# rongzhao-zhang/EfficientQ

Hardware: AMD Instinct MI355X
Metric: ptq_calibration_throughput (higher is better)
Workload: dtype i8xi8->i32 (exact) for the Gram systems and per-iteration loss convs of the layers with quantised input, f32/f64 elsewhere

## Files before the change

### efficientq_amd/_lib.py

```python
from __future__ import annotations

import ctypes as C
import os

import torch

_HERE = os.path.dirname(os.path.abspath(__file__))
LIB_PATH = os.path.join(_HERE, "libeffq_hip.so")

EFFQ_OK = 0
_ERR_NAMES = {1: "EFFQ_ERR_ARG", 2: "EFFQ_ERR_HIP", 3: "EFFQ_ERR_WORKSPACE", 4: "EFFQ_ERR_NO_DEVICE",
              5: "EFFQ_ERR_NOT_CONVERGED"}


class EffqError(RuntimeError):
    pass


class Geom(C.Structure):
    _fields_ = [(n, C.c_int32) for n in
                ("N", "C1", "C2", "D", "H", "W", "KD", "KH", "KW", "SD", "SH", "SW", "PD", "PH", "PW")]

    def out_dims(self):
        return ((self.D + 2 * self.PD - self.KD) // self.SD + 1,
# ... 79 lines not shown
    "effq_fixed_point_coop_rec": (_I, [_P, _P, _P, _SZ, _I, _D, _D, _D, _I, _P, _P, _P, _P]),
    "effq_fp_check": (_I, [_P, _P, _P]),
    "effq_fp_channels_max_row": (_I, []),
    "effq_fixed_point_channels": (_I, [_P, _P, _P, _I, _I, _I, _D, _I, _P, _P, _P, _P]),
    "effq_fixed_point_channels_proj": (_I, [_P, _P, _P, _I, _I, _I, _D, _I, _P, _P, _P, _P, _F, _P, _P, _P, _I, _I, _D,
                                            _D, _P]),
    "effq_gram_packed_elems": (_SZ, [_I, _I]),
    "effq_gram_pack": (_I, [_P, _P, _I, _I, _P, _P]),
    "effq_gram_unpack": (_I, [_P, _I, _I, _P, _P, _P]),
    "effq_act_quant_backward": (_I, [_P, _P, _I, _P, _P, _P, _SZ, _P, _P]),
    "effq_att_classes_ws_bytes": (_SZ, []),
    "effq_att_classes": (_I, [_P, _LL, _P, _P, _P, C.POINTER(C.c_int32), _P, _P]),
    "effq_prof_enable": (_I, [_I]),
    "effq_prof_count": (_I, []),
    "effq_prof_read": (_I, [_I, C.POINTER(ProfRecord)]),
    "effq_admm_num_inverses": (_I, [_D, _D, _I, _I]),
    "effq_admm_run": (_I, [C.POINTER(AdmmRunArgs)]),
    "effq_admm_select_best": (_I, [_P, _I, _P, _P, _SZ, _SZ, _P, _P, _P, _P]),
    "effq_gram_ws_bytes": (_SZ, [_GP, _I]),
    "effq_gram_accum": (_I, [_P, _P, _P, _GP, _I, _P, _P, _I, _P, _SZ, _P]),
    "effq_gram_plan_query": (_I, [_GP, _I, _IP, _IP, _IP, _IP, _LLP, _IP, _IP]),
    "effq_gram_i8_supported": (_I, [_GP, _I]),
    "effq_gram_i8_ws_bytes": (_SZ, [_GP, _I]),
    "effq_gram_accum_i8": (_I, [_P, _P, _GP, _I, _P, _I, _P, _P, _P, _I, _LL, _P, _P, _I, _P, _SZ, _P]),
    "effq_gram_accum_i8_unw": (_I, [_P, _P, _GP, _I, _P, _I, _P, _P, _P, _I, _LL, _P, _P, _I, _P, _P, _P, _SZ, _P]),
    "effq_gram_i8_plan_query": (_I, [_GP, _I, _LL, _IP, _IP, _IP, _IP, _IP, _IP]),
    "effq_upsample_trilinear": (_I, [_P, _I, _I, _I, _I, _I, _I, _I, _I, _P, _P]),
    "effq_gram_f64_supported": (_I, [_GP, _I]),
    "effq_gram_f64_ws_bytes": (_SZ, [_GP, _I]),
    "effq_gram_f64": (_I, [_P, _P, _GP, _I, _P, _P, _P, _SZ, _P]),
    "effq_gram_f64_plan_query": (_I, [_GP, _I, _IP, _IP, _IP, _IP]),
    "effq_gram_loss_ws_bytes": (_SZ, [_I]),
    "effq_gram_loss": (_I, [_P, _P, _P, _P, _P, _I, _I, _I, _P, _P, _SZ, _P]),
    "effq_packed_bytes": (_SZ, [_SZ, _I]),
    "effq_pack_levels": (_I, [_P, _SZ, _I, _P, _P]),
    "effq_unpack_levels": (_I, [_P, _SZ, _I, _P, _P]),
    "effq_ainv_ld": (_I, [_I]),
    "effq_fp_bracket_export_words": (_SZ, []),
    "effq_fp_bracket_export": (_I, [_P, _SZ, _P, _P, _SZ, _P]),
    "effq_fp_bracket_rebase": (_I, [_P, _P, _SZ, _P]),
    "effq_fp_bracket_import": (_I, [_P, _SZ, _P, _I, _SZ, _P, _P, _SZ, _P]),
    "effq_admm_uses_traj": (_I, [_SZ, _I]),
    "effq_gram_loss_i8_supported": (_I, [_I, _I, _I, _I]),
    "effq_gram_loss_i8_num_planes": (_I, [C.c_longlong]),
    "effq_gram_loss_i8_planes_bytes": (_SZ, [_I, _I, _I]),
    "effq_gram_loss_i8_prepare": (_I, [_P, _I, _I, _P, _I, _I, _P, _P, _P]),
    "effq_gram_loss_i8_ws_bytes": (_SZ, []),
    "effq_gram_loss_i8": (_I, [_P, _I, _P, _P, _P, _P, _P, _P, _P, _I, _I, _I, _I, _I, _I, _P, _P, _SZ, _P]),
    "effq_spd_inverse_ws_bytes": (_SZ, [_I]),
    "effq_spd_inverse": (_I, [_P, _I, _I, _D, _D, _P, _P, _SZ, _P]),
    "effq_spd_inverse_plan": (_I, [_I, _IP, _IP, _IP]),
    "effq_prox_plan_query": (_I, [_I, _I, _IP, _IP, _IP, _IP]),
    "effq_prox_ws_bytes": (_SZ, [_I, _I]),
    "effq_prox_solve": (_I, [_P, _P, _P, _P, _P, _P, _I, _I, _I, _D, _D, _P, _P, _P, _SZ, _P]),
    "effq_prox_solve_shifted": (_I, [_P, _P, _P, _P, _P, _P, _I, _I, _I, _D, _D, _D, _I, _P, _P, _P, _SZ, _P]),
    "effq_admm_presum": (_I, [_P, _P, _P, _SZ, _P]),
    "effq_admm_project_dual": (_I, [_P, _P, _P, _I, _P, _P, _F, _P, _SZ, _P]),
    "effq_conv_i8_supported": (_I, [_GP, _I, _I]),
    "effq_conv_i8s_supported": (_I, [_GP, _I, _I]),
    "effq_conv_i8s_ws_bytes": (_SZ, [_GP, _I, _I]),
    "conv3d_calib_step_i8s": (_I, [_P, _P, _P, _P, _GP, _P, _I, _P, _I, _I, _P, _P, _SZ, _P]),
    "effq_conv_i8_ws_bytes": (_SZ, [_GP]),
    "conv3d_calib_step_i8": (_I, [_P, _P, _P, _P, _GP, _P, _I, _P, _I, _P, _P, _SZ, _P]),
    "effq_conv_i8_out_supported": (_I, [_GP, _I, _I]),
    "conv3d_quant_forward_i8": (_I, [_P, _P, _P, _P, _P, _GP, _P, _I, _P, _I, _P, _P, _P, _SZ, _P]),
    "effq_conv_ws_bytes": (_SZ, [_GP]),
# ... 56 lines not shown
```

### efficientq_amd/csrc/admm_run.hip

```cpp
#include <stdlib.h>
#include <algorithm>
#include <vector>
#include "common.h"
#include "internal.h"
#include "project_dual.h"

namespace effq {

struct ProfRec {
  int kind, iter, loss_kind, c2, n;
  effq_geom geom;
  hipEvent_t e0, e1;
};
static thread_local std::vector<ProfRec> g_prof;
static thread_local int g_prof_every = 0;
enum { PROF_PROX = 1, PROF_FIXED_POINT = 2, PROF_PROJECT = 3, PROF_LOSS = 4, PROF_INVERSE = 5, PROF_WAIT = 6 };

struct ProfScope {
  bool on;
  hipStream_t stream;
  ProfRec rec;
  ProfScope(bool enabled, int kind, int iter, const effq_admm_run_args* a, hipStream_t st) : on(enabled), stream(st) {
    if (!on) return;
    rec.kind = kind;
    rec.iter = iter;
    rec.loss_kind = a->loss_kind;
    rec.c2 = a->c2;
    rec.n = a->n;
    rec.geom = a->geom;
    if (hipEventCreate(&rec.e0) != hipSuccess || hipEventCreate(&rec.e1) != hipSuccess) {
      on = false;
      return;
    }
    (void)hipEventRecord(rec.e0, stream);
  }
  void close() {
    if (!on) return;
    (void)hipEventRecord(rec.e1, stream);
    g_prof.push_back(rec);
    on = false;
  }
};

constexpr int ADMM_MAX_RHOS = 16;

struct RhoPlan {
  int count;
  double rho[ADMM_MAX_RHOS];
  int first_iter[ADMM_MAX_RHOS];
  bool shifted_first;
  bool overflow;
};

static RhoPlan plan_rhos(double rho, double rho_max, int iters, int period) {
  RhoPlan p;
  p.count = 0;
  p.overflow = false;
  double r = rho;
// ... 293 lines not shown
                                        a->alpha_ring + (size_t)it.i * p.c2,
                                        a->w_iters_ring ? a->w_iters_ring + (size_t)it.i * p.c2 : nullptr, a->err_flag,
                                        it.G, it.dual_div, it.next_rhs ? p.bm : nullptr, a->B0, a->W0, p.n, p.bm_ld,
                                        it.rho_next, a->eta, p.s_main);
  else if (kind == FpKind::traj && it.parts != nullptr)
    rc = effq_fixed_point_traj_parts(it.parts, it.parts_n, it.parts_ld, p.c2, nwrow, p.has_b, a->dual, a->wstar, it.bstar,
                                     a->v, a->w_levels, -1.0, 1.0, a->tol, maxit, it.st, a->fp_pred, a->fp_traj_ws,
                                     a->fp_traj_ws_bytes, p.s_main);
  else if (kind == FpKind::traj)
    rc = effq_fixed_point_traj(a->wstar, a->dual, a->v, p.nw, a->w_levels, -1.0, 1.0, a->tol, maxit, it.st, a->fp_pred,
                               a->fp_traj_ws, a->fp_traj_ws_bytes, p.s_main);
  else if (kind == FpKind::bucket)
    rc = effq_fixed_point_bucket_rec(a->wstar, a->dual, a->v, p.nw, a->w_levels, -1.0, 1.0, a->tol, maxit, it.st, a->fp_ws,
                                     a->fp_ws_bytes, rec, p.s_main);
  else if (kind == FpKind::small)
    rc = effq_fixed_point_small_fused(a->wstar, a->dual, a->v, p.nw, a->w_levels, -1.0, 1.0, a->tol, maxit, it.st,
                                      fuse_proj ? &pf : nullptr, p.s_main);
  else
    rc = effq_fixed_point_coop_rec(a->wstar, a->dual, a->v, p.nw, a->w_levels, -1.0, 1.0, a->tol, maxit, it.st, a->red_ws,
                                   rec, p.s_main);
  if (rc != EFFQ_OK) return rc;
  p_fp.close();
  *bm_ready = it.next_rhs;
  if (fuse_proj) return EFFQ_OK;
  ProfScope p_pr(it.prof, PROF_PROJECT, it.i, a, p.s_main);
  rc = effq_project_dual_impl(a->v, a->wstar, it.st, a->w_levels, it.G, a->dual, it.dual_div, it.Gq, p.nw, a->err_flag,
                              nxp, p.s_main);
  if (rc != EFFQ_OK) return rc;
  p_pr.close();
  return EFFQ_OK;
}

static int enqueue_losses(const effq_admm_run_args* a, const AdmmPlan& p, int j0, int i) {
  const int step = a->loss_kind == 5 ? 16 : 1;
  for (int j = j0; j <= i; j += step) {
    const int cnt = (i - j + 1 < step) ? (i - j + 1) : step;
    const float* Gj = a->G_ring + (size_t)j * p.nw;
    const int8_t* Gqj = a->Gq_ring ? a->Gq_ring + (size_t)j * p.nw : nullptr;
    const float* bj = p.has_b ? a->b_ring + (size_t)j * p.c2 : nullptr;
    const effq_fp_state* stj = a->state_ring + j;
    double* sq = a->hist + 2 * (size_t)j;
    const bool prof = g_prof_every > 0 && (a->loss_kind == 5 ? (j / p.loss_group) % 2 == 1 :
                      !(p.rhos.shifted_first && j == 0) && (j % g_prof_every) == g_prof_every / 2);
    ProfScope p_loss(prof, PROF_LOSS, j, a, p.s_loss);
    int rc;
    if (a->loss_kind == 5)
      rc = effq_gram_loss_i8(a->loss_planes, a->loss_nplanes, a->loss_Au, a->loss_Bu, a->loss_syy, Gqj, bj, stj,
                             a->act_alpha_dev, a->act_levels, a->w_levels, p.c2, p.n, p.has_b, cnt, sq, a->conv_ws,
                             a->conv_ws_bytes, p.s_loss);
    else if (a->loss_kind == 1)
      rc = conv3d_calib_step_i8(a->xidx, Gqj, bj, a->y_fp, &a->geom, a->act_alpha_dev, a->act_levels, stj, a->w_levels,
                                sq, a->conv_ws, a->conv_ws_bytes, p.s_loss);
    else if (a->loss_kind == 2)
      rc = conv3d_calib_step_i8s(a->xidx, Gqj, bj, a->y_fp, &a->geom, a->act_alpha_dev, a->act_levels, stj, a->w_levels,
                                 j == 0 ? 1 : 0, sq, a->conv_ws, a->conv_ws_bytes, p.s_loss);
    else if (a->loss_kind == 4)
      rc = effq_gram_loss(a->loss_Au, a->loss_Bu, a->loss_syy, Gj, bj, p.c2, p.n, p.has_b, sq, a->conv_ws,
                          a->conv_ws_bytes, p.s_loss);
    else
      rc = conv3d_quant_calib_step(a->xq, Gj, bj, a->y_fp, nullptr, &a->geom, nullptr, 0, sq, nullptr, a->conv_ws,
                                   a->conv_ws_bytes, p.s_loss);
    if (rc != EFFQ_OK) return rc;
    p_loss.close();
  }
  return EFFQ_OK;
}

}
using namespace effq;

extern "C" {

int effq_admm_uses_traj(size_t nw, int w_levels) {
  constexpr int traj_levels = 4;
  constexpr size_t traj_min = 65536;
  return (w_levels <= traj_levels && nw >= traj_min && nw <= effq_fp_traj_max()) ? 1 : 0;
}

int effq_admm_num_inverses(double rho, double rho_max, int iters, int period) {
  if (!(rho > 0.0) || iters <= 0 || period <= 0) return -1;
  const RhoPlan p = plan_rhos(rho, rho_max, iters, period);
  if (p.overflow) return -1;
  return p.count - (p.shifted_first ? 1 : 0);
}

int effq_admm_run(const effq_admm_run_args* a) {
  AdmmPlan p;
  if (const int rc = admm_plan(a, &p); rc != EFFQ_OK) return rc;
  constexpr int LOSS_EVENTS = 4;
  EventPool events;
  EFFQ_HIP(events.open());
// ... 74 lines not shown

int effq_gram_unpack(const float* buf, int n, int c2, float* A0, float* B0, void* stream) {
  EFFQ_CHECK_ARG(A0 && B0 && buf && n > 0 && c2 > 0);
  size_t blocks = ((size_t)n * n + (size_t)c2 * n + 255) / 256;
  if (blocks > 8192) blocks = 8192;
  hipLaunchKernelGGL(k_gram_unpack, dim3((unsigned)blocks), dim3(256), 0, as_stream(stream), buf, n, c2, A0, B0);
  EFFQ_LAUNCH_CHECK();
  return EFFQ_OK;
}

int effq_prof_enable(int every) {
  for (ProfRec& r : g_prof) {
    (void)hipEventDestroy(r.e0);
    (void)hipEventDestroy(r.e1);
  }
  g_prof.clear();
  g_prof_every = every > 0 ? every : 0;
  return EFFQ_OK;
}

int effq_prof_count(void) { return (int)g_prof.size(); }

int effq_prof_read(int i, effq_prof_record* out) {
  EFFQ_CHECK_ARG(out != nullptr && i >= 0 && i < (int)g_prof.size());
  const ProfRec& r = g_prof[(size_t)i];
  float ms = 0.0f;
  EFFQ_HIP(hipEventElapsedTime(&ms, r.e0, r.e1));
  out->kind = r.kind;
  out->iter = r.iter;
  out->loss_kind = r.loss_kind;
  out->c2 = r.c2;
  out->n = r.n;
  out->geom = r.geom;
  out->ms = ms;
  return EFFQ_OK;
}

int effq_admm_select_best(const double* hist, int iters, const float* G_ring, const float* b_ring, size_t nw, size_t nb,
                          float* best_G, float* best_b, double* best_out, void* stream) {
  EFFQ_CHECK_ARG(hist && G_ring && best_G && best_out && iters > 0 && nw > 0);
  EFFQ_CHECK_ARG((b_ring == nullptr) == (best_b == nullptr));
  size_t blocks = (nw + 255) / 256;
  if (blocks > 1024) blocks = 1024;
  hipLaunchKernelGGL(k_select_best, dim3((unsigned)blocks), dim3(256), 0, as_stream(stream), hist, iters, G_ring, b_ring,
                     nw, nb, best_G, best_b, best_out);
  EFFQ_LAUNCH_CHECK();
  return EFFQ_OK;
}

}
```

### efficientq_amd/csrc/gram_loss.hip

```cpp
#include "common.h"

namespace effq {

constexpr int GL_TB = 64;
constexpr int GL_T = 256;
constexpr int GL_CC = 32;

struct GramLossParams {
  const double* Au;
  const double* Bu;
  const double* syy;
  const float* G;
  const float* b;
  int c2, n, has_bias, nt;
  int ntile, ncross;
  double* partials;
  unsigned int* ticket;
  double* out;
};

__device__ __forceinline__ float gl_g(const GramLossParams& p, int c, int k) {
  const int nw = p.n - p.has_bias;
  if (k < nw) return p.G[(size_t)c * nw + k];
  return (k < p.n && p.b != nullptr) ? p.b[c] : 0.0f;
}

__global__ __launch_bounds__(GL_T) void k_gram_loss(GramLossParams p) {
  __shared__ float gk[GL_CC][GL_TB + 4], gj[GL_CC][GL_TB + 4];
  __shared__ double red_smem[16];
  __shared__ int s_last;
  const int tid = threadIdx.x;
  double part = 0.0;
  if ((int)blockIdx.x < p.ntile) {
    int K = 0, rem = (int)blockIdx.x;
    while (rem >= p.nt - K) {
      rem -= p.nt - K;
      ++K;
    }
    const int J = K + rem;
    const int k0 = K * GL_TB, j0 = J * GL_TB;
    const int tk = (tid >> 4) * 4, tj = (tid & 15) * 4;
    double m[4][4];
#pragma unroll
    for (int a = 0; a < 4; ++a)
#pragma unroll
      for (int b = 0; b < 4; ++b) m[a][b] = 0.0;
    for (int c0 = 0; c0 < p.c2; c0 += GL_CC) {
      __syncthreads();
      for (int e = tid; e < GL_CC * GL_TB; e += GL_T) {
        const int c = e / GL_TB, q = e % GL_TB;
        const bool cok = c0 + c < p.c2;
        gk[c][q] = cok ? gl_g(p, c0 + c, k0 + q) : 0.0f;
        gj[c][q] = cok ? gl_g(p, c0 + c, j0 + q) : 0.0f;
      }
      __syncthreads();
#pragma unroll 4
      for (int c = 0; c < GL_CC; ++c) {
        double a4[4], b4[4];
#pragma unroll
        for (int a = 0; a < 4; ++a) {
          a4[a] = (double)gk[c][tk + a];
          b4[a] = (double)gj[c][tj + a];
        }
#pragma unroll
        for (int a = 0; a < 4; ++a)
#pragma unroll
          for (int b = 0; b < 4; ++b) m[a][b] = __builtin_fma(a4[a], b4[b], m[a][b]);
      }
    }
    double acc = 0.0;
#pragma unroll
    for (int a = 0; a < 4; ++a) {
      const int k = k0 + tk + a;
#pragma unroll
      for (int b = 0; b < 4; ++b) {
        const int j = j0 + tj + b;
        if (k < p.n && j < p.n) acc = __builtin_fma(p.Au[(size_t)k * p.n + j], m[a][b], acc);
      }
    }
    part = (J > K) ? 2.0 * acc : acc;
  } else {
    const int w = (int)blockIdx.x - p.ntile;
    const size_t tot = (size_t)p.c2 * p.n;
    double acc = 0.0;
    for (size_t e = (size_t)w * GL_T + tid; e < tot; e += (size_t)p.ncross * GL_T) {
      const int c = (int)(e / p.n), k = (int)(e % p.n);
      acc = __builtin_fma((double)gl_g(p, c, k), p.Bu[e], acc);
    }
    part = -2.0 * acc;
  }
  double v[1] = {part};
  grid_sum_finish<1>(v, p.partials, p.ticket, p.out, red_smem, &s_last);
  if (s_last && tid == 0) {
    const double loss = p.out[0] + *p.syy;
    p.out[0] = loss;
    p.out[1] = loss;
  }
}

}
using namespace effq;

extern "C" {

size_t effq_gram_loss_ws_bytes(int n) {
  if (n <= 0) return 0;
  const size_t nt = ((size_t)n + GL_TB - 1) / GL_TB;
  return 256 + (nt * (nt + 1) / 2 + 64) * sizeof(double) + 256;
}

int effq_gram_loss(const double* Au, const double* Bu, const double* syy_dev, const float* G, const float* b, int c2, int n,
                   int has_bias, double* sqerr_out, void* ws, size_t ws_bytes, void* stream) {
  EFFQ_CHECK_ARG(Au && Bu && syy_dev && G && sqerr_out && ws && c2 > 0 && n > 0);
  EFFQ_CHECK_ARG(!has_bias || b != nullptr);
  if (ws_bytes < effq_gram_loss_ws_bytes(n)) {
    set_error("gram_loss: workspace %zu < required %zu", ws_bytes, effq_gram_loss_ws_bytes(n));
    return EFFQ_ERR_WORKSPACE;
  }
  GramLossParams p;
  p.Au = Au; p.Bu = Bu; p.syy = syy_dev; p.G = G; p.b = has_bias ? b : nullptr;
  p.c2 = c2; p.n = n; p.has_bias = has_bias ? 1 : 0;
  p.nt = (n + GL_TB - 1) / GL_TB;
  p.ntile = p.nt * (p.nt + 1) / 2;
  size_t nc = ((size_t)c2 * n + (size_t)GL_T * 8 - 1) / ((size_t)GL_T * 8);
  if (nc < 1) nc = 1;
  if (nc > 64) nc = 64;
  p.ncross = (int)nc;
  EFFQ_CHECK_ARG(p.ntile + p.ncross <= RED_MAX_BLOCKS * 16);
  char* base = reinterpret_cast<char*>(ws);
  p.ticket = reinterpret_cast<unsigned int*>(base);
  p.partials = reinterpret_cast<double*>(base + 256);
  p.out = sqerr_out;
  hipLaunchKernelGGL(k_gram_loss, dim3((unsigned)(p.ntile + p.ncross)), dim3(GL_T), 0, as_stream(stream), p);
  EFFQ_LAUNCH_CHECK();
  return EFFQ_OK;
}

}
```

### efficientq_amd/hip_ops.py

```python
from __future__ import annotations

import ctypes as C
import math
from typing import Optional, Tuple

import torch

from . import _lib
from ._lib import Geom, check

ADMM_TOL = 1e-5
FP_BRACKET_MIN = 1 << 18
DP_GATHER_AFTER = 4
DP_GATHER_MAX_BYTES = 128 << 20


def _ptr(t: Optional[torch.Tensor]):
    return None if t is None else C.c_void_p(t.data_ptr())


def to_ndhwc(x: torch.Tensor) -> torch.Tensor:
    return x.permute(0, 2, 3, 4, 1).contiguous()


# ... 423 lines not shown
        return bool(self.lib.effq_gram_f64_supported(C.byref(geom), int(has_bias)))

    def gram_f64(self, x_ndhwc: torch.Tensor, y_ndhwc: torch.Tensor, geom: Geom, has_bias: bool):
        x, y = self._f32(x_ndhwc), self._f32(y_ndhwc)
        _check_shapes(geom, x, y=y)
        n = geom.C1 * geom.KD * geom.KH * geom.KW + int(has_bias)
        Au = torch.empty(n, n, dtype=torch.float64, device=self.device)
        Bu = torch.empty(geom.C2, n, dtype=torch.float64, device=self.device)
        ws = self._workspace("gram_f64", self.lib.effq_gram_f64_ws_bytes(C.byref(geom), int(has_bias)))
        check(self.lib.effq_gram_f64(_ptr(x), _ptr(y), C.byref(geom), int(has_bias), _ptr(Au), _ptr(Bu), _ptr(ws),
                                     ws.numel(), self.stream), "effq_gram_f64")
        return Au, Bu

    def upsample_trilinear(self, x_ndhwc: torch.Tensor, scale) -> torch.Tensor:
        x = self._f32(x_ndhwc)
        N, D, H, W, Cc = (int(i) for i in x.shape)
        sd, sh, sw = (int(i) for i in scale)
        out = torch.empty(N, D * sd, H * sh, W * sw, Cc, dtype=torch.float32, device=self.device)
        check(self.lib.effq_upsample_trilinear(_ptr(x), N, D, H, W, Cc, sd, sh, sw, _ptr(out), self.stream),
              "effq_upsample_trilinear")
        return out

    def gram_loss(self, Au: torch.Tensor, Bu: torch.Tensor, syy: torch.Tensor, G: torch.Tensor, b, sqerr=None):
        c2, n = (int(i) for i in Bu.shape)
        has_b = b is not None
        if (Au.dtype != torch.float64 or Bu.dtype != torch.float64 or syy.dtype != torch.float64 or
                tuple(Au.shape) != (n, n) or G.numel() != c2 * (n - int(has_b))):
            raise _lib.EffqError("gram_loss: operand shapes / dtypes do not match")
        if sqerr is None:
            sqerr = torch.zeros(2, dtype=torch.float64, device=self.device)
        ws = self._workspace("gram_loss", self.lib.effq_gram_loss_ws_bytes(n))
        check(self.lib.effq_gram_loss(_ptr(Au), _ptr(Bu), _ptr(syy), _ptr(self._f32(G)), _ptr(b), c2, n, int(has_b),
                                      _ptr(sqerr), _ptr(ws), ws.numel(), self.stream), "effq_gram_loss")
        return sqerr

    def gram_loss_i8_supported(self, c2: int, n: int, has_b: bool, w_levels: int) -> bool:
        return bool(self.lib.effq_gram_loss_i8_supported(int(c2), int(n), int(has_b), int(w_levels)))

    def gram_loss_i8_planes(self, Au: torch.Tensor, has_b: bool, act_alpha: torch.Tensor, act_levels: int, voxels: int):
        n = int(Au.shape[0])
        P = self.lib.effq_gram_loss_i8_num_planes(int((act_levels - 1) ** 2 * voxels))
        if P < 1:
            return None
        nw = n - int(has_b)
        planes = torch.empty(P, (nw + 255) // 256 * 256, nw, dtype=torch.int8, device=self.device)
        assert planes.numel() == self.lib.effq_gram_loss_i8_planes_bytes(n, int(has_b), P)
        err = torch.zeros(1, dtype=torch.int32, device=self.device)
        al = self._f32(act_alpha.reshape(1))
        check(self.lib.effq_gram_loss_i8_prepare(_ptr(Au), n, int(has_b), _ptr(al), int(act_levels), P, _ptr(planes),
                                                 _ptr(err), self.stream), "effq_gram_loss_i8_prepare")
        planes._effq_err = err
        return planes

    def gram_loss_i8(self, planes, Au, Bu, syy, Gq, b, states, act_alpha, act_levels: int, w_levels: int, hist=None):
        count, c2 = int(Gq.shape[0]), int(Bu.shape[0])
        n = int(Bu.shape[1])
        has_b = b is not None
        if hist is None:
            hist = torch.zeros(count, 2, dtype=torch.float64, device=self.device)
        ws = self._workspace("gram_loss_i8", self.lib.effq_gram_loss_i8_ws_bytes())
        al = self._f32(act_alpha.reshape(1))
        check(self.lib.effq_gram_loss_i8(_ptr(planes), int(planes.shape[0]), _ptr(Au), _ptr(Bu), _ptr(syy), _ptr(Gq), _ptr(b),
                                         _ptr(states), _ptr(al), int(act_levels), int(w_levels), c2, n, int(has_b), count,
                                         _ptr(hist), _ptr(ws), ws.numel(), self.stream), "effq_gram_loss_i8")
        return hist

# ... 99 lines not shown
        dev, f32 = self.device, torch.float32
        ld = self.lib.effq_ainv_ld(n)
        r = SimpleNamespace(iters=int(iters), nw=nw, c2=c2, has_b=has_b, channel_wise=bool(channel_wise))
        r.ainv = torch.empty(n_inv, n, ld, dtype=f32, device=dev)
        r.dual = torch.empty(nw, dtype=f32, device=dev)
        r.wstar = torch.empty(nw, dtype=f32, device=dev)
        r.v = torch.empty(nw, dtype=f32, device=dev)
        r.G_ring = torch.empty(iters, nw, dtype=f32, device=dev)
        r.Gq_ring = torch.empty(iters, nw, dtype=torch.int8, device=dev) if loss_kind in (1, 2, 5) else None
        r.b_ring = torch.empty(iters, c2, dtype=f32, device=dev) if has_b else None
        r.state_ring = torch.zeros(iters, 5, dtype=torch.float64, device=dev)
        r.hist = torch.zeros(iters, 2, dtype=torch.float64, device=dev)
        r.err = torch.zeros(1, dtype=torch.int32, device=dev)
        r.res = torch.zeros(iters, 2, dtype=torch.float64, device=dev) if residuals else None
        r.alpha_ring = torch.zeros(iters, c2, dtype=torch.float64, device=dev) if channel_wise else None
        r.w_iters_ring = torch.zeros(iters, c2, dtype=torch.int32, device=dev) if channel_wise else None
        main = torch.cuda.current_stream(dev)
        loss_s = self.loss_stream() if overlap else None
        side_s = self.side_stream()
        prox = self._workspace("prox", self.lib.effq_prox_ws_bytes(c2, n))
        inv = self._workspace("inv", self.lib.effq_spd_inverse_ws_bytes(n))
        inv_side = (self._workspace("inv_side", self.lib.effq_spd_inverse_ws_bytes(n))
                    if n_inv > 1 else None)
        inv_side2 = (self._workspace("inv_side2", self.lib.effq_spd_inverse_ws_bytes(n))
                     if n_inv > 2 else None)
        fpw = (self._workspace("fp_bucket", self.lib.effq_fp_bucket_ws_bytes(nw))
               if nw <= self.lib.effq_fp_bucket_max() and not channel_wise else None)
        traj = not channel_wise and bool(self.lib.effq_admm_uses_traj(nw, int(levels)))
        tws = self._workspace("fp_traj", self.lib.effq_fp_traj_ws_bytes(nw)) if traj else None
        r.fp_pred = torch.zeros(self.lib.effq_fp_traj_pred_bytes(), dtype=torch.uint8, device=dev) if traj else None
        if loss_kind == 5:
            cws = self._workspace("gram_loss_i8", self.lib.effq_gram_loss_i8_ws_bytes())
        elif loss_kind == 4:
            cws = self._workspace("gram_loss", self.lib.effq_gram_loss_ws_bytes(n))
        elif loss_kind == 1:
            cws = self._workspace("conv_i8", self.lib.effq_conv_i8_ws_bytes(C.byref(geom)))
        elif loss_kind == 2:
            cws = self._workspace("conv_i8s", self.lib.effq_conv_i8s_ws_bytes(C.byref(geom), int(act_levels),
                                                                             int(levels)))
        else:
            cws = self._workspace("conv", self.lib.effq_conv_ws_bytes(C.byref(geom)))
        al = self._f32(act_alpha.reshape(1)) if (act_alpha is not None and loss_kind in (1, 2, 5)) else None
        a = _lib.AdmmRunArgs()
        p = lambda t: None if t is None else t.data_ptr()
        a.A0, a.B0, a.W0, a.b0 = p(A0), p(B0), p(W0), p(b0)
        a.c2, a.n, a.has_bias, a.w_levels = c2, n, int(has_b), int(levels)
        a.iters, a.rho_period = int(iters), int(period)
        a.rho, a.rho_max, a.eta, a.tol = float(rho), float(rho_max), float(eta), ADMM_TOL
        a.geom = geom
        a.loss_kind, a.act_levels = int(loss_kind), int(act_levels)
        a.xq = p(xq) if loss_kind == 0 else None
        a.xidx = p(xidx) if loss_kind in (1, 2) else None
        if loss_kind in (4, 5):
            Au, Bu, syy = loss_gram
            if (Au.dtype != torch.float64 or Bu.dtype != torch.float64 or syy.dtype != torch.float64 or
                    tuple(Au.shape) != (n, n) or tuple(Bu.shape) != (c2, n) or syy.numel() != 1):
                raise _lib.EffqError("admm_run: loss_gram wants fp64 (Au [n,n], Bu [c2,n], syy [1])")
            a.loss_Au, a.loss_Bu, a.loss_syy = p(Au), p(Bu), p(syy)
            if loss_kind == 5:
                a.loss_planes, a.loss_nplanes = p(planes), int(planes.shape[0])
                r.loss_planes = planes
        a.y_fp, a.act_alpha_dev = p(y), p(al)
        a.dual, a.wstar, a.v = p(r.dual), p(r.wstar), p(r.v)
        a.G_ring, a.Gq_ring, a.b_ring = p(r.G_ring), p(r.Gq_ring), p(r.b_ring)
        a.state_ring, a.hist, a.err_flag = p(r.state_ring), p(r.hist), p(r.err)
        a.res_ring = p(r.res)
        a.channel_wise, a.alpha_ring, a.w_iters_ring = int(bool(channel_wise)), p(r.alpha_ring), p(r.w_iters_ring)
# ... 500 lines not shown
```

### include/effq_hip.h

```cpp
#ifndef EFFQ_HIP_H
#define EFFQ_HIP_H

#include <stddef.h>
#include <stdint.h>

#ifdef __cplusplus
extern "C" {
#endif

enum {
  EFFQ_OK = 0,
  EFFQ_ERR_ARG = 1,
  EFFQ_ERR_HIP = 2,
  EFFQ_ERR_WORKSPACE = 3,
  EFFQ_ERR_NO_DEVICE = 4,
  EFFQ_ERR_NOT_CONVERGED = 5
};

typedef struct effq_geom {
  int32_t N, C1, C2;
  int32_t D, H, W;
  int32_t KD, KH, KW;
  int32_t SD, SH, SW;
  int32_t PD, PH, PW;
// ... 80 lines not shown
                                   double rho_next, double eta, void* stream);

int effq_fp_check(const effq_fp_state* state_dev, int32_t* err_flag_dev, void* stream);

size_t effq_gram_ws_bytes(const effq_geom* g, int has_bias);
int effq_gram_accum(const float* x_ndhwc, const float* att, const float* y_ndhwc, const effq_geom* g,
                    int has_bias, float* A0, float* B0, int accumulate, void* ws, size_t ws_bytes,
                    void* stream);
int effq_gram_plan_query(const effq_geom* g, int has_bias, int* vec, int* nb, int* npairs, int* nsplit,
                         long long* vox_per_split, int* fold, int* finish_blocks);

int effq_gram_i8_supported(const effq_geom* g, int act_levels);
size_t effq_gram_i8_ws_bytes(const effq_geom* g, int ncls);
int effq_gram_accum_i8(const uint8_t* xidx_ndhwc, const float* y_ndhwc, const effq_geom* g, int has_bias,
                       const float* act_alpha_dev, int act_levels, const int32_t* vox_list,
                       const int32_t* chunk_cls, const float* cls_w_dev, int ncls, long long n_list,
                       float* A0, float* B0, int accumulate, void* ws, size_t ws_bytes, void* stream);
int effq_gram_accum_i8_unw(const uint8_t* xidx_ndhwc, const float* y_ndhwc, const effq_geom* g, int has_bias,
                           const float* act_alpha_dev, int act_levels, const int32_t* vox_list, const int32_t* chunk_cls,
                           const float* cls_w_dev, int ncls, long long n_list, float* A0, float* B0, int accumulate,
                           double* Au, double* Bu, void* ws, size_t ws_bytes, void* stream);
int effq_gram_i8_plan_query(const effq_geom* g, int ncls, long long n_list, int* nb, int* nbx, int* npairs, int* nchunks,
                            int* cps, int* nsplit);

int effq_gram_f64_supported(const effq_geom* g, int has_bias);
size_t effq_gram_f64_ws_bytes(const effq_geom* g, int has_bias);
int effq_gram_f64(const float* x_ndhwc, const float* y_ndhwc, const effq_geom* g, int has_bias, double* Au, double* Bu,
                  void* ws, size_t ws_bytes, void* stream);
int effq_gram_f64_plan_query(const effq_geom* g, int has_bias, int* nchunk, int* grid, int* ntiles, int* tpw);

size_t effq_gram_loss_ws_bytes(int n);
int effq_gram_loss(const double* Au, const double* Bu, const double* syy_dev, const float* G, const float* b, int c2, int n,
                   int has_bias, double* sqerr_out, void* ws, size_t ws_bytes, void* stream);

int effq_gram_loss_i8_supported(int c2, int n, int has_bias, int w_levels);
int effq_gram_loss_i8_num_planes(long long kmax);
size_t effq_gram_loss_i8_planes_bytes(int n, int has_bias, int nplanes);
int effq_gram_loss_i8_prepare(const double* Au, int n, int has_bias, const float* act_alpha_dev, int act_levels,
                              int nplanes, int8_t* planes, int32_t* err_flag_dev, void* stream);
size_t effq_gram_loss_i8_ws_bytes(void);
int effq_gram_loss_i8(const int8_t* planes, int nplanes, const double* Au, const double* Bu, const double* syy_dev,
                      const int8_t* Gq, const float* b, const effq_fp_state* states, const float* act_alpha_dev,
                      int act_levels, int w_levels, int c2, int n, int has_bias, int count, double* hist_out, void* ws,
                      size_t ws_bytes, void* stream);


size_t effq_att_classes_ws_bytes(void);
int effq_att_classes(const float* att, long long V, int32_t* vox_list, int32_t* chunk_cls, float* cls_w_dev,
                     int32_t* info_host_out, void* ws, void* stream);

int effq_spd_inverse_prepare(void* stream);
int effq_ainv_ld(int n);
size_t effq_spd_inverse_ws_bytes(int n);
int effq_spd_inverse(const float* A0, int n, int has_bias, double rho, double eta, float* Ainv,
                     void* ws, size_t ws_bytes, void* stream);
int effq_spd_inverse_plan(int n, int* wide, int* nblk, int* pivot_blocks);

size_t effq_prox_ws_bytes(int c2, int n);
int effq_prox_solve(const float* B0, const float* Ainv, const float* W0, const float* b0, const float* G,
                    const float* dual, int c2, int n, int has_bias, double rho, double eta, float* wstar,
                    float* bstar, void* ws, size_t ws_bytes, void* stream);
int effq_prox_plan_query(int c2, int n, int* variant, int* gx, int* gy, int* nsplit);

int effq_prox_solve_shifted(const float* B0, const float* Ainv, const float* W0, const float* b0, const float* G,
                            const float* dual, int c2, int n, int has_bias, double rho, double eta,
                            double rho_inv, int nterms, float* wstar, float* bstar, void* ws, size_t ws_bytes,
// ... 143 lines not shown
```

Before: 24.77.

## Batch f64 Gram loss over up to 16 iterations using MFMA f64 tiles

```diff
diff --git a/efficientq_amd/_lib.py b/efficientq_amd/_lib.py
--- a/efficientq_amd/_lib.py
+++ b/efficientq_amd/_lib.py
@@ -135,6 +135,8 @@
     "effq_gram_f64_plan_query": (_I, [_GP, _I, _IP, _IP, _IP, _IP]),
     "effq_gram_loss_ws_bytes": (_SZ, [_I]),
     "effq_gram_loss": (_I, [_P, _P, _P, _P, _P, _I, _I, _I, _P, _P, _SZ, _P]),
+    "effq_gram_loss_group_ws_bytes": (_SZ, [_I, _I]),
+    "effq_gram_loss_group": (_I, [_P, _P, _P, _P, _P, _I, _I, _I, _I, _P, _P, _SZ, _P]),
     "effq_packed_bytes": (_SZ, [_SZ, _I]),
     "effq_pack_levels": (_I, [_P, _SZ, _I, _P, _P]),
     "effq_unpack_levels": (_I, [_P, _SZ, _I, _P, _P]),
diff --git a/efficientq_amd/csrc/admm_run.hip b/efficientq_amd/csrc/admm_run.hip
--- a/efficientq_amd/csrc/admm_run.hip
+++ b/efficientq_amd/csrc/admm_run.hip
@@ -9,6 +9,7 @@
 
 struct ProfRec {
   int kind, iter, loss_kind, c2, n;
+  int div;
   effq_geom geom;
   hipEvent_t e0, e1;
 };
@@ -24,6 +25,7 @@
     if (!on) return;
     rec.kind = kind;
     rec.iter = iter;
+    rec.div = 1;
     rec.loss_kind = a->loss_kind;
     rec.c2 = a->c2;
     rec.n = a->n;
@@ -383,7 +385,9 @@
 }
 
 static int enqueue_losses(const effq_admm_run_args* a, const AdmmPlan& p, int j0, int i) {
-  const int step = a->loss_kind == 5 ? 16 : 1;
+  int step = (a->loss_kind == 4 || a->loss_kind == 5) ? 16 : 1;
+  if (a->loss_kind == 4)
+    while (step > 1 && a->conv_ws_bytes < effq_gram_loss_group_ws_bytes(p.n, step)) --step;
   for (int j = j0; j <= i; j += step) {
     const int cnt = (i - j + 1 < step) ? (i - j + 1) : step;
     const float* Gj = a->G_ring + (size_t)j * p.nw;
@@ -391,9 +395,13 @@
     const float* bj = p.has_b ? a->b_ring + (size_t)j * p.c2 : nullptr;
     const effq_fp_state* stj = a->state_ring + j;
     double* sq = a->hist + 2 * (size_t)j;
-    const bool prof = g_prof_every > 0 && (a->loss_kind == 5 ? (j / p.loss_group) % 2 == 1 :
-                      !(p.rhos.shifted_first && j == 0) && (j % g_prof_every) == g_prof_every / 2);
+    bool prof = false;
+    if (g_prof_every > 0 && a->loss_kind == 5) prof = (j / p.loss_group) % 2 == 1;
+    else if (g_prof_every > 0)
+      for (int jj = j; jj < j + cnt; ++jj)
+        prof = prof || (!(p.rhos.shifted_first && jj == 0) && (jj % g_prof_every) == g_prof_every / 2);
     ProfScope p_loss(prof, PROF_LOSS, j, a, p.s_loss);
+    if (a->loss_kind == 4) p_loss.rec.div = cnt;
     int rc;
     if (a->loss_kind == 5)
       rc = effq_gram_loss_i8(a->loss_planes, a->loss_nplanes, a->loss_Au, a->loss_Bu, a->loss_syy, Gqj, bj, stj,
@@ -406,8 +414,8 @@
       rc = conv3d_calib_step_i8s(a->xidx, Gqj, bj, a->y_fp, &a->geom, a->act_alpha_dev, a->act_levels, stj, a->w_levels,
                                  j == 0 ? 1 : 0, sq, a->conv_ws, a->conv_ws_bytes, p.s_loss);
     else if (a->loss_kind == 4)
-      rc = effq_gram_loss(a->loss_Au, a->loss_Bu, a->loss_syy, Gj, bj, p.c2, p.n, p.has_b, sq, a->conv_ws,
-                          a->conv_ws_bytes, p.s_loss);
+      rc = effq_gram_loss_group(a->loss_Au, a->loss_Bu, a->loss_syy, Gj, bj, p.c2, p.n, p.has_b, cnt, sq, a->conv_ws,
+                                a->conv_ws_bytes, p.s_loss);
     else
       rc = conv3d_quant_calib_step(a->xq, Gj, bj, a->y_fp, nullptr, &a->geom, nullptr, 0, sq, nullptr, a->conv_ws,
                                    a->conv_ws_bytes, p.s_loss);
@@ -548,7 +556,7 @@
   out->c2 = r.c2;
   out->n = r.n;
   out->geom = r.geom;
-  out->ms = ms;
+  out->ms = ms / (float)r.div;
   return EFFQ_OK;
 }
 
diff --git a/efficientq_amd/csrc/gram_loss.hip b/efficientq_amd/csrc/gram_loss.hip
--- a/efficientq_amd/csrc/gram_loss.hip
+++ b/efficientq_amd/csrc/gram_loss.hip
@@ -1,10 +1,15 @@
 #include "common.h"
 
 namespace effq {
+
+typedef double f64x4 __attribute__((ext_vector_type(4)));
 
 constexpr int GL_TB = 64;
 constexpr int GL_T = 256;
 constexpr int GL_CC = 32;
+constexpr int GL_LD = 80;
+constexpr int GL_MAX_CNT = 16;
+constexpr int GL_MAX_CROSS = 64;
 
 struct GramLossParams {
   const double* Au;
@@ -14,23 +19,25 @@
   const float* b;
   int c2, n, has_bias, nt;
   int ntile, ncross;
+  int cnt;
   double* partials;
   unsigned int* ticket;
   double* out;
 };
 
-__device__ __forceinline__ float gl_g(const GramLossParams& p, int c, int k) {
+enum { GL_WEIGHT = 0, GL_BIAS = 1, GL_ZERO = 2 };
+__device__ __forceinline__ int gl_kind(const GramLossParams& p, int k) {
   const int nw = p.n - p.has_bias;
-  if (k < nw) return p.G[(size_t)c * nw + k];
-  return (k < p.n && p.b != nullptr) ? p.b[c] : 0.0f;
+  return k < nw ? GL_WEIGHT : (k < p.n && p.b != nullptr) ? GL_BIAS : GL_ZERO;
 }
 
 __global__ __launch_bounds__(GL_T) void k_gram_loss(GramLossParams p) {
-  __shared__ float gk[GL_CC][GL_TB + 4], gj[GL_CC][GL_TB + 4];
-  __shared__ double red_smem[16];
+  __shared__ float gk[GL_CC * GL_LD], gj[GL_CC * GL_LD];
+  __shared__ double wsum[GL_MAX_CNT][GL_T / 64];
   __shared__ int s_last;
-  const int tid = threadIdx.x;
-  double part = 0.0;
+  const int tid = threadIdx.x, lane = tid & 63, wid = tid >> 6;
+  const int nw = p.n - p.has_bias;
+  const size_t gstride = (size_t)p.c2 * nw;
   if ((int)blockIdx.x < p.ntile) {
     int K = 0, rem = (int)blockIdx.x;
     while (rem >= p.nt - K) {
@@ -38,64 +45,144 @@
       ++K;
     }
     const int J = K + rem;
+    const bool diag = J == K;
     const int k0 = K * GL_TB, j0 = J * GL_TB;
-    const int tk = (tid >> 4) * 4, tj = (tid & 15) * 4;
-    double m[4][4];
-#pragma unroll
-    for (int a = 0; a < 4; ++a)
-#pragma unroll
-      for (int b = 0; b < 4; ++b) m[a][b] = 0.0;
-    for (int c0 = 0; c0 < p.c2; c0 += GL_CC) {
-      __syncthreads();
-      for (int e = tid; e < GL_CC * GL_TB; e += GL_T) {
-        const int c = e / GL_TB, q = e % GL_TB;
-        const bool cok = c0 + c < p.c2;
-        gk[c][q] = cok ? gl_g(p, c0 + c, k0 + q) : 0.0f;
-        gj[c][q] = cok ? gl_g(p, c0 + c, j0 + q) : 0.0f;
-      }
-      __syncthreads();
+    const int wr = wid >> 1, wc = wid & 1, lr = lane & 15, lk = lane >> 4;
+    double au[2][2][4];
+    const double sym = diag ? 1.0 : 2.0;
+#pragma unroll
+    for (int mi = 0; mi < 2; ++mi)
+#pragma unroll
+      for (int ni = 0; ni < 2; ++ni)
+#pragma unroll
+        for (int r = 0; r < 4; ++r) {
+          const int k = k0 + wr * 32 + mi * 16 + lk + 4 * r, j = j0 + wc * 32 + ni * 16 + lr;
+          au[mi][ni][r] = (k < p.n && j < p.n) ? sym * p.Au[(size_t)k * p.n + j] : 0.0;
+        }
+    const int q = lane;
+    const int kq = k0 + q, jq = j0 + q;
+    const int kkind = gl_kind(p, kq), jkind = gl_kind(p, jq);
+    float pk[GL_CC / 4], pj[GL_CC / 4];
+    auto fetch = [&](int it, int c0) {
+      const float* Gs = p.G + (size_t)it * gstride;
+      const float* bs = p.b != nullptr ? p.b + (size_t)it * p.c2 : nullptr;
+#pragma unroll
+      for (int i = 0; i < GL_CC / 4; ++i) {
+        const int c = c0 + wid + 4 * i;
+        const bool cok = c < p.c2;
+        pk[i] = !cok ? 0.0f : kkind == GL_WEIGHT ? Gs[(size_t)c * nw + kq] : kkind == GL_BIAS ? bs[c] : 0.0f;
+        if (!diag) pj[i] = !cok ? 0.0f : jkind == GL_WEIGHT ? Gs[(size_t)c * nw + jq] : jkind == GL_BIAS ? bs[c] : 0.0f;
+      }
+    };
+    const float* As = gk + wr * 32 + lr;
+    const float* Bs = (diag ? gk : gj) + wc * 32 + lr;
+    f64x4 m[2][2];
+#pragma unroll
+    for (int mi = 0; mi < 2; ++mi)
+#pragma unroll
+      for (int ni = 0; ni < 2; ++ni)
+#pragma unroll
+        for (int r = 0; r < 4; ++r) m[mi][ni][r] = 0.0;
+    fetch(0, 0);
+    int it = 0, c0 = 0;
+    for (;;) {
+      lds_barrier();
+#pragma unroll
+      for (int i = 0; i < GL_CC / 4; ++i) {
+        gk[(wid + 4 * i) * GL_LD + q] = pk[i];
+        if (!diag) gj[(wid + 4 * i) * GL_LD + q] = pj[i];
+      }
+      int itn = it, cn = c0 + GL_CC;
+      if (cn >= p.c2) {
+        cn = 0;
+        ++itn;
+      }
+      const bool more = itn < p.cnt;
+      if (more) fetch(itn, cn);
+      lds_barrier();
 #pragma unroll 4
-      for (int c = 0; c < GL_CC; ++c) {
-        double a4[4], b4[4];
-#pragma unroll
-        for (int a = 0; a < 4; ++a) {
-          a4[a] = (double)gk[c][tk + a];
-          b4[a] = (double)gj[c][tj + a];
-        }
-#pragma unroll
-        for (int a = 0; a < 4; ++a)
-#pragma unroll
-          for (int b = 0; b < 4; ++b) m[a][b] = __builtin_fma(a4[a], b4[b], m[a][b]);
-      }
-    }
-    double acc = 0.0;
-#pragma unroll
-    for (int a = 0; a < 4; ++a) {
-      const int k = k0 + tk + a;
-#pragma unroll
-      for (int b = 0; b < 4; ++b) {
-        const int j = j0 + tj + b;
-        if (k < p.n && j < p.n) acc = __builtin_fma(p.Au[(size_t)k * p.n + j], m[a][b], acc);
-      }
-    }
-    part = (J > K) ? 2.0 * acc : acc;
+      for (int ks = 0; ks < GL_CC / 4; ++ks) {
+        double a[2], b[2];
+#pragma unroll
+        for (int mi = 0; mi < 2; ++mi) a[mi] = (double)As[(ks * 4 + lk) * GL_LD + mi * 16];
+#pragma unroll
+        for (int ni = 0; ni < 2; ++ni) b[ni] = (double)Bs[(ks * 4 + lk) * GL_LD + ni * 16];
+#pragma unroll
+        for (int mi = 0; mi < 2; ++mi)
+#pragma unroll
+          for (int ni = 0; ni < 2; ++ni) m[mi][ni] = __builtin_amdgcn_mfma_f64_16x16x4f64(a[mi], b[ni], m[mi][ni], 0, 0, 0);
+      }
+      if (cn == 0) {
+        double acc = 0.0;
+#pragma unroll
+        for (int mi = 0; mi < 2; ++mi)
+#pragma unroll
+          for (int ni = 0; ni < 2; ++ni)
+#pragma unroll
+            for (int r = 0; r < 4; ++r) {
+              acc = __builtin_fma(au[mi][ni][r], m[mi][ni][r], acc);
+              m[mi][ni][r] = 0.0;
+            }
+        acc = wave_sum(acc);
+        if (lane == 0) wsum[it][wid] = acc;
+      }
+      if (!more) break;
+      it = itn;
+      c0 = cn;
+    }
   } else {
     const int w = (int)blockIdx.x - p.ntile;
-    const size_t tot = (size_t)p.c2 * p.n;
+    for (int it = 0; it < p.cnt; ++it) {
+      const float* Gs = p.G + (size_t)it * gstride;
+      double acc = 0.0;
+      for (int c = w; c < p.c2; c += p.ncross) {
+        const float* g = Gs + (size_t)c * nw;
+        const double* bu = p.Bu + (size_t)c * p.n;
+        for (int k = tid; k < nw; k += GL_T) acc = __builtin_fma((double)g[k], bu[k], acc);
+        if (tid == 0 && p.b != nullptr) acc = __builtin_fma((double)p.b[(size_t)it * p.c2 + c], bu[nw], acc);
+      }
+      acc = wave_sum(-2.0 * acc);
+      if (lane == 0) wsum[it][wid] = acc;
+    }
+  }
+  const unsigned int nblk = gridDim.x;
+  __syncthreads();
+  if (wid == 0) {
+    if (tid < p.cnt) {
+      double t = 0.0;
+      for (int wv = 0; wv < GL_T / 64; ++wv) t += wsum[tid][wv];
+      p.partials[(size_t)tid * nblk + blockIdx.x] = t;
+    }
+    __builtin_amdgcn_fence(__ATOMIC_RELEASE, "agent");
+    asm volatile("s_waitcnt vmcnt(0)" ::: "memory");
+    if (tid == 0) {
+      const unsigned int t = __hip_atomic_fetch_add(p.ticket, 1u, __ATOMIC_RELAXED, __HIP_MEMORY_SCOPE_AGENT);
+      s_last = (t == nblk - 1) ? 1 : 0;
+    }
+  }
+  __syncthreads();
+  if (!s_last) return;
+  if (tid == 0) {
+    __builtin_amdgcn_fence(__ATOMIC_ACQUIRE, "agent");
+    asm volatile("s_waitcnt vmcnt(0)" ::: "memory");
+  }
+  __syncthreads();
+  for (int it = 0; it < p.cnt; ++it) {
+    const double* part = p.partials + (size_t)it * nblk;
     double acc = 0.0;
-    for (size_t e = (size_t)w * GL_T + tid; e < tot; e += (size_t)p.ncross * GL_T) {
-      const int c = (int)(e / p.n), k = (int)(e % p.n);
-      acc = __builtin_fma((double)gl_g(p, c, k), p.Bu[e], acc);
-    }
-    part = -2.0 * acc;
-  }
-  double v[1] = {part};
-  grid_sum_finish<1>(v, p.partials, p.ticket, p.out, red_smem, &s_last);
-  if (s_last && tid == 0) {
-    const double loss = p.out[0] + *p.syy;
-    p.out[0] = loss;
-    p.out[1] = loss;
-  }
+    for (unsigned int b = tid; b < nblk; b += GL_T) acc += __hip_atomic_load(&part[b], __ATOMIC_RELAXED, __HIP_MEMORY_SCOPE_AGENT);
+    acc = wave_sum(acc);
+    if (lane == 0) wsum[it][wid] = acc;
+  }
+  __syncthreads();
+  if (tid < p.cnt) {
+    double t = 0.0;
+    for (int wv = 0; wv < GL_T / 64; ++wv) t += wsum[tid][wv];
+    const double loss = t + *p.syy;
+    p.out[2 * tid] = loss;
+    p.out[2 * tid + 1] = loss;
+  }
+  if (tid == 0) __hip_atomic_store(p.ticket, 0u, __ATOMIC_RELAXED, __HIP_MEMORY_SCOPE_AGENT);
 }
 
 }
@@ -103,18 +190,21 @@
 
 extern "C" {
 
-size_t effq_gram_loss_ws_bytes(int n) {
-  if (n <= 0) return 0;
+size_t effq_gram_loss_group_ws_bytes(int n, int cnt) {
+  if (n <= 0 || cnt <= 0) return 0;
   const size_t nt = ((size_t)n + GL_TB - 1) / GL_TB;
-  return 256 + (nt * (nt + 1) / 2 + 64) * sizeof(double) + 256;
-}
-
-int effq_gram_loss(const double* Au, const double* Bu, const double* syy_dev, const float* G, const float* b, int c2, int n,
-                   int has_bias, double* sqerr_out, void* ws, size_t ws_bytes, void* stream) {
+  return 256 + (nt * (nt + 1) / 2 + GL_MAX_CROSS) * (size_t)cnt * sizeof(double) + 256;
+}
+
+size_t effq_gram_loss_ws_bytes(int n) { return effq_gram_loss_group_ws_bytes(n, 1); }
+
+int effq_gram_loss_group(const double* Au, const double* Bu, const double* syy_dev, const float* G, const float* b, int c2,
+                         int n, int has_bias, int cnt, double* sqerr_out, void* ws, size_t ws_bytes, void* stream) {
   EFFQ_CHECK_ARG(Au && Bu && syy_dev && G && sqerr_out && ws && c2 > 0 && n > 0);
   EFFQ_CHECK_ARG(!has_bias || b != nullptr);
-  if (ws_bytes < effq_gram_loss_ws_bytes(n)) {
-    set_error("gram_loss: workspace %zu < required %zu", ws_bytes, effq_gram_loss_ws_bytes(n));
+  EFFQ_CHECK_ARG(cnt >= 1 && cnt <= GL_MAX_CNT);
+  if (ws_bytes < effq_gram_loss_group_ws_bytes(n, cnt)) {
+    set_error("gram_loss: workspace %zu < required %zu", ws_bytes, effq_gram_loss_group_ws_bytes(n, cnt));
     return EFFQ_ERR_WORKSPACE;
   }
   GramLossParams p;
@@ -122,10 +212,8 @@
   p.c2 = c2; p.n = n; p.has_bias = has_bias ? 1 : 0;
   p.nt = (n + GL_TB - 1) / GL_TB;
   p.ntile = p.nt * (p.nt + 1) / 2;
-  size_t nc = ((size_t)c2 * n + (size_t)GL_T * 8 - 1) / ((size_t)GL_T * 8);
-  if (nc < 1) nc = 1;
-  if (nc > 64) nc = 64;
-  p.ncross = (int)nc;
+  p.ncross = c2 < GL_MAX_CROSS ? c2 : GL_MAX_CROSS;
+  p.cnt = cnt;
   EFFQ_CHECK_ARG(p.ntile + p.ncross <= RED_MAX_BLOCKS * 16);
   char* base = reinterpret_cast<char*>(ws);
   p.ticket = reinterpret_cast<unsigned int*>(base);
@@ -136,4 +224,9 @@
   return EFFQ_OK;
 }
 
-}
+int effq_gram_loss(const double* Au, const double* Bu, const double* syy_dev, const float* G, const float* b, int c2, int n,
+                   int has_bias, double* sqerr_out, void* ws, size_t ws_bytes, void* stream) {
+  return effq_gram_loss_group(Au, Bu, syy_dev, G, b, c2, n, has_bias, 1, sqerr_out, ws, ws_bytes, stream);
+}
+
+}
diff --git a/efficientq_amd/hip_ops.py b/efficientq_amd/hip_ops.py
--- a/efficientq_amd/hip_ops.py
+++ b/efficientq_amd/hip_ops.py
@@ -479,6 +479,26 @@
         ws = self._workspace("gram_loss", self.lib.effq_gram_loss_ws_bytes(n))
         check(self.lib.effq_gram_loss(_ptr(Au), _ptr(Bu), _ptr(syy), _ptr(self._f32(G)), _ptr(b), c2, n, int(has_b),
                                       _ptr(sqerr), _ptr(ws), ws.numel(), self.stream), "effq_gram_loss")
+        return sqerr
+
+    def gram_loss_group(self, Au: torch.Tensor, Bu: torch.Tensor, syy: torch.Tensor, G: torch.Tensor, b, sqerr=None):
+        c2, n = (int(i) for i in Bu.shape)
+        has_b = b is not None
+        cnt = int(G.shape[0])
+        G = self._f32(G)
+        if has_b:
+            b = self._f32(b)
+        if (Au.dtype != torch.float64 or Bu.dtype != torch.float64 or syy.dtype != torch.float64 or
+                tuple(Au.shape) != (n, n) or G.numel() != cnt * c2 * (n - int(has_b)) or
+                (has_b and b.numel() != cnt * c2)):
+            raise _lib.EffqError("gram_loss_group: operand shapes / dtypes do not match")
+        if sqerr is None:
+            sqerr = torch.zeros(cnt, 2, dtype=torch.float64, device=self.device)
+        elif sqerr.dtype != torch.float64 or sqerr.numel() < 2 * cnt or not sqerr.is_contiguous():
+            raise _lib.EffqError("gram_loss_group: sqerr must hold [cnt, 2] contiguous float64")
+        ws = self._workspace("gram_loss", self.lib.effq_gram_loss_group_ws_bytes(n, cnt))
+        check(self.lib.effq_gram_loss_group(_ptr(Au), _ptr(Bu), _ptr(syy), _ptr(G), _ptr(b), c2, n, int(has_b), cnt,
+                                            _ptr(sqerr), _ptr(ws), ws.numel(), self.stream), "effq_gram_loss_group")
         return sqerr
 
     def gram_loss_i8_supported(self, c2: int, n: int, has_b: bool, w_levels: int) -> bool:
@@ -644,7 +664,7 @@
         if loss_kind == 5:
             cws = self._workspace("gram_loss_i8", self.lib.effq_gram_loss_i8_ws_bytes())
         elif loss_kind == 4:
-            cws = self._workspace("gram_loss", self.lib.effq_gram_loss_ws_bytes(n))
+            cws = self._workspace("gram_loss", self.lib.effq_gram_loss_group_ws_bytes(n, 16))
         elif loss_kind == 1:
             cws = self._workspace("conv_i8", self.lib.effq_conv_i8_ws_bytes(C.byref(geom)))
         elif loss_kind == 2:
diff --git a/include/effq_hip.h b/include/effq_hip.h
--- a/include/effq_hip.h
+++ b/include/effq_hip.h
@@ -136,6 +136,9 @@
 size_t effq_gram_loss_ws_bytes(int n);
 int effq_gram_loss(const double* Au, const double* Bu, const double* syy_dev, const float* G, const float* b, int c2, int n,
                    int has_bias, double* sqerr_out, void* ws, size_t ws_bytes, void* stream);
+size_t effq_gram_loss_group_ws_bytes(int n, int cnt);
+int effq_gram_loss_group(const double* Au, const double* Bu, const double* syy_dev, const float* G, const float* b, int c2,
+                         int n, int has_bias, int cnt, double* sqerr_out, void* ws, size_t ws_bytes, void* stream);
 
 int effq_gram_loss_i8_supported(int c2, int n, int has_bias, int w_levels);
 int effq_gram_loss_i8_num_planes(long long kmax);
```

Result: no change. 24.84, median of 2 (+0.3%).
